# COMPiLELab/krylov_robustness

Measured on AMD Instinct MI355X. Metric: trace(exp(A)) evals/sec + achieved HBM GB/s, n=1M nnz=10M, 1/2/4/8 GPU, higher is better.
Workload: dtype f64

## Files before the change

__graft_entry__.py:

```python
from __future__ import annotations

import os
import subprocess
import sys

ROOT = os.path.dirname(os.path.abspath(__file__))


def build() -> None:
    jobs = str(min(16, os.cpu_count() or 4))
    subprocess.run(["make", "-j", jobs, "-C", os.path.join(ROOT, "krylov_robustness_amd", "csrc")],
                   check=True)
    subprocess.run(["make", "-C", os.path.join(ROOT, "oracle")], check=True)
    subprocess.run(["make", "-j", jobs, "-C", os.path.join(ROOT, "tests", "mexstub")], check=True)
    wave_check = os.path.join(ROOT, "tests", "native", "wave_check")
    if os.path.isfile(os.path.join(wave_check, "Makefile")):
        subprocess.run(["make", "-C", wave_check], check=True)
    if ROOT not in sys.path:
        sys.path.insert(0, ROOT)
    import krylov_robustness_amd as kra
    from krylov_robustness_amd import _lib
    _lib.load()
    assert kra.LIB_PATH.endswith("libkrylov_hip.so")


def smoke() -> None:
    if ROOT not in sys.path:
        sys.path.insert(0, ROOT)
    import numpy as np
    import scipy.sparse as sp

    import krylov_robustness_amd as kra
    from oracle import slq_ref

    z = np.load(os.path.join(ROOT, "tests", "golden", "graphs.npz"))
    n = int(z["oregon_A0__n"][0])
    A = sp.csr_matrix((z["oregon_A0__data"], z["oregon_A0__indices"], z["oregon_A0__indptr"]),
                      shape=(n, n))
    ctx = kra.Context(0)
    D = kra.DeviceMatrix(A, ctx)
    s1, _, q = kra.slq_quadforms(D, 32, 20, seed=7, fun="exp", ctx=ctx)
    _, q_ref = slq_ref.slq_trace(A, 32, 20, seed=7, fun="exp")
    err = float(np.max(np.abs(q - q_ref) / np.abs(q_ref)))
    if not err < 1e-8:
        raise AssertionError(f"smoke: GPU vs oracle max rel err {err:.3e}")
    print(f"smoke ok: tr(exp(A)) ~ {s1 / 32:.6e} (32 probes, m=20), max rel err vs oracle {err:.2e}")


if __name__ == "__main__":
    build()
# ... 3 lines not shown
```

krylov_robustness_amd/csrc/kt_internal.h:

```cpp
#pragma once
#include <algorithm>
#include <hip/hip_runtime.h>
#include <stdint.h>

#include <string>
#include <vector>

#include "../../include/krylov_trace.h"

struct kt_matrix_s;

#ifndef KT_DIAG
#define KT_DIAG 0
#endif

namespace kt {

void set_error(const std::string& msg);

struct Status {
    int code;
    std::string msg;
};

// ... 154 lines not shown
};

}

struct kt_context_s {
    int device = 0;
    hipStream_t stream = nullptr;
    hipStream_t aux_stream[3] = {nullptr, nullptr, nullptr};
    int num_cu = 256;
    bool profile = false;
    int k1_flags = 8;
    bool k2_nt = true;
    int64_t yform_redone = 0;
    int64_t fu_dense = 0;
    int64_t fu_last_cols = 0;
    int64_t expmv_calls = 0;
    int64_t expmv_terms = 0;
    int ky_flags = 8;
    bool yform = true;
    void* blas = nullptr;
    kt_context_s* helper = nullptr;
    void* workers[3] = {nullptr, nullptr, nullptr};
    void (*workers_free)(void*) = nullptr;
    kt::ProfSlot prof[kt::PROF_NSLOTS];
    kt::Workspace ws;
    kt::ScratchPool pool;
};

namespace kt {
struct DevCSR {
    int* rowptr = nullptr;
    int* col = nullptr;
    double* val = nullptr;
    int* long_rows = nullptr;
    int n_long = 0;
    int n_heavy = 0;
    int* med_rows = nullptr;
    int n_med = 0;
    int* short_tasks = nullptr;
    int n_short = 0;
    int* med_tasks = nullptr;
    int* perm = nullptr;
    int *ck_beg = nullptr, *ck_end = nullptr, *sp_rows = nullptr, *sp_first = nullptr;
    int n_chunks = 0, n_split = 0;
    bool built = false;
    char* blob = nullptr;
    size_t blob_bytes = 0;
    PinnedBuf stage;
    void release();
    void invalidate() { built = false; }
};
}

struct kt_matrix_s {
    kt_context_s* ctx = nullptr;
    int64_t n = 0, nnz = 0;
    int long_thresh = 64;
    bool unit_values = false;
    int symmetric = -1;
    kt::DevCSR hub;
    std::vector<int32_t> new2old, old2new;
    kt::DevCSR nat;
    std::vector<int64_t> h_rowptr;
    std::vector<int32_t> h_col;
    std::vector<double> h_val;
    uint64_t version = 0;
// ... 39 lines not shown
```

krylov_robustness_amd/csrc/kt_kernels.hip:

```cpp
#include <hip/hip_runtime.h>

#include "kt_launch.h"
#include "kt_wave.h"
#include <stdint.h>

#include <cstdlib>

#include <type_traits>

namespace kt {

__device__ __forceinline__ uint64_t sm64(uint64_t x) {
    uint64_t z = x + 0x9E3779B97F4A7C15ULL;
    z = (z ^ (z >> 30)) * 0xBF58476D1CE4E5B9ULL;
    z = (z ^ (z >> 27)) * 0x94D049BB133111EBULL;
    return z ^ (z >> 31);
}

template <int P, int VW> struct GeoW {
    static constexpr int VEC = VW;
    static constexpr int LPR = P / VEC;
    static constexpr int GPW = 64 / LPR;
};
template <int P> using Geo = GeoW<P, (P >= 2) ? 2 : 1>;
// ... 354 lines not shown
        guard[p] = 1.0;
    } else {
        const double aj = ys[0 * P + p], bj = ys[1 * P + p], am1 = ys[2 * P + p];
        const double nyj = ys[3 * P + p], ydj = ys[4 * P + p], b1 = ys[5 * P + p];
        g = guard[p];
        const double b1sq = b1 * b1;
        an = (d0 - 2.0 * aj * nyj - 2.0 * bj * ydj + aj * aj * aj + 2.0 * aj * bj * bj + bj * bj * am1) /
             b1sq;
        ny2 = d2;
        bn = b1;
        bnext_sq = ny2 - an * an - b1sq;
        ys[1 * P + p] = b1;
        ys[2 * P + p] = aj;
        ys[4 * P + p] = d1;
    }
    const double bnext = sqrt(fmax(bnext_sq, 0.0));
    ys[0 * P + p] = an;
    ys[3 * P + p] = ny2;
    ys[5 * P + p] = bnext;
    t_alpha[p] = an;
    t_up[p] = bn;
    t_low[p] = bnext;
    if (!last) {
        const double ratio = bnext_sq / ny2;
        guard[p] = (ratio < g || !(ratio == ratio)) ? ratio : g;
    }
    const bool ok = bnext > 0.0 && bnext < INFINITY;
    const double inv = ok ? 1.0 / bnext : 0.0;
    ys[6 * P + p] = inv;
    ys[7 * P + p] = an * inv;
    ys[8 * P + p] = bn * inv;
}

template <int P, int FLAGS, class G = Geo<P>>
__device__ __forceinline__ void row_epilogue_y(int row, int p0, const double* s, const double* cg,
                                               const double* ca, const double* cb, bool has_old,
                                               const double* __restrict__ X,
                                               const double* __restrict__ Yold,
                                               double* __restrict__ Out, double* d0, double* d1,
                                               double* d2, __amdgpu_buffer_rsrc_t orsrc,
                                               const double* __restrict__ Vc = nullptr,
                                               const double* __restrict__ Vo = nullptr,
                                               double* __restrict__ Vn = nullptr, int bcols = 0) {
    using V = VecT<G::VEC>;
    const int64_t off = (int64_t)row * P + p0;
    const typename V::T xi = V::load(X + off);
    if constexpr (FLAGS & KF_VB) {
        if (p0 < bcols) {
            const typename V::T vc = V::load(Vc + off);
            typename V::T vo;
            if (Vo) vo = V::load(Vo + off);
#pragma unroll
            for (int e = 0; e < G::VEC; ++e) {
                double v = fma(-ca[e], V::get(vc, e), cg[e] * V::get(xi, e));
                if (Vo) v = fma(-cb[e], V::get(vo, e), v);
                if (p0 + e < bcols) Vn[off + e] = v;
            }
        }
    }
    if (!Out) {
#pragma unroll
        for (int e = 0; e < G::VEC; ++e) d0[e] = fma(V::get(xi, e), s[e], d0[e]);
        return;
    }
    typename V::T yo;
    if (has_old) yo = V::load_nt(Yold + off);
    typename V::T o;
    double* op = reinterpret_cast<double*>(&o);
#pragma unroll
    for (int e = 0; e < G::VEC; ++e) {
        const double x = V::get(xi, e);
        double u = fma(-ca[e], x, cg[e] * s[e]);
        if (has_old) u = fma(-cb[e], V::get(yo, e), u);
        op[e] = u;
        d0[e] = fma(x, s[e], d0[e]);
        d1[e] = fma(x, u, d1[e]);
        d2[e] = fma(u, u, d2[e]);
    }
    if constexpr (FLAGS & KF_SC1) store_sc1<G::VEC>(orsrc, (uint32_t)(off * 8), op);
    else if constexpr (FLAGS & KF_NTY) V::store_nt(Out + off, o);
    else V::store(Out + off, o);
}

template <int P, class G>
__device__ __forceinline__ double sign_of(uint32_t w, int p0, int e) {
    return ((w >> ((p0 + e) & 31)) & 1u) ? -1.0 : 1.0;
}
template <int P, int FLAGS, class G>
__device__ __forceinline__ void row_gather_signs(int k0, int end, int stride, int p0,
                                                 const int* __restrict__ col,
                                                 const double* __restrict__ val,
                                                 const uint32_t* __restrict__ S, double* s) {
    constexpr int W = (P + 31) / 32;
    const int wo = p0 >> 5;
    int k = k0;
    for (; k + 3 * stride < end; k += 4 * stride) {
        const int c0 = ld_stream<FLAGS>(col + k), c1 = ld_stream<FLAGS>(col + k + stride);
// ... 172 lines not shown
            if (end - beg > long_thresh) continue;
            double s[G::VEC];
#pragma unroll
            for (int e = 0; e < G::VEC; ++e) s[e] = 0.0;
            gather_row<P, FLAGS, G>(beg, end, 1, p0, col, val, X, s);
            row_epilogue_y<P, FLAGS, G>(row, p0, s, cg, ca, cb, has_old, X, Yold, Out, d0, d1, d2,
                                        orsrc, Vc, Vo, Vn, bcols);
        }
    }

#pragma unroll
    for (int o = G::LPR; o < 64; o <<= 1)
#pragma unroll
        for (int e = 0; e < G::VEC; ++e) {
            d0[e] += kt::shfl_xor(d0[e], o);
            d1[e] += kt::shfl_xor(d1[e], o);
            d2[e] += kt::shfl_xor(d2[e], o);
        }
    __shared__ double red[WAVES][3][P];
    if (grp == 0) {
#pragma unroll
        for (int e = 0; e < G::VEC; ++e) {
            red[wave][0][p0 + e] = d0[e];
            red[wave][1][p0 + e] = d1[e];
            red[wave][2][p0 + e] = d2[e];
        }
    }
    __syncthreads();
    for (int t = threadIdx.x; t < 3 * P; t += BLOCK) {
        const int q = t / P, p = t % P;
        double v = 0.0;
#pragma unroll
        for (int w = 0; w < WAVES; ++w) v += red[w][q][p];
        partial[(int64_t)t * gridDim.x + blockIdx.x] = v;
    }
}

template <int P, int BLOCK, int FLAGS>
__global__ __launch_bounds__(BLOCK) void k_spmm_block(
    const int* __restrict__ row_ptr, const int* __restrict__ col, const double* __restrict__ val,
    int n, const double* __restrict__ X, int ldx, double* __restrict__ Y, int ldy,
    const int* __restrict__ long_rows, int n_long, int long_thresh, int long_blocks,
    const int* __restrict__ skip, const int* __restrict__ ck_beg, const int* __restrict__ ck_end,
    int n_chunks, int chunk_blocks, int split_thresh, double* __restrict__ ck_part) {
    using G = GeoB<P>;
    using V = VecT<G::VEC>;
    constexpr int WAVES = BLOCK / 64;
    if (skip && *skip == 0) return;
    X += (int64_t)blockIdx.y * P;
    Y += (int64_t)blockIdx.y * P;
    const int lane = threadIdx.x & 63;
    const int wave = threadIdx.x >> 6;
    const int sub = lane % G::LPR;
    const int grp = lane / G::LPR;
    const int p0 = sub * G::VEC;
    if ((int)blockIdx.x < chunk_blocks) {
        double* part = ck_part + (int64_t)blockIdx.y * n_chunks * P;
        for (int ci = blockIdx.x * WAVES + wave; ci < n_chunks; ci += chunk_blocks * WAVES) {
            double s[G::VEC];
#pragma unroll
            for (int e = 0; e < G::VEC; ++e) s[e] = 0.0;
            gather_row<P, FLAGS, G>(ck_beg[ci] + grp, ck_end[ci], G::GPW, p0, col, val, X, s, ldx);
#pragma unroll
            for (int o = G::LPR; o < 64; o <<= 1)
#pragma unroll
                for (int e = 0; e < G::VEC; ++e) s[e] += kt::shfl_xor(s[e], o);
// ... 1191 lines not shown


hipError_t launch_spmm_lanczos(int P, int flags, int grid, const int* rp, const int* ci,
                               const double* va, int n, const double* X, const double* Yold,
                               double* Out, const double* coef, double* partial,
                               const int* long_rows, int n_long, int long_thresh, int long_blocks,
                               hipStream_t st, const double* Vc, const double* Vo, double* Vn, int bcols) {
    return dispatch_p(P, [&](auto c) {
        constexpr int PP = decltype(c)::value;
#define KT_KY(F)                                                                                   \
    k_spmm_lanczos<PP, kBlock, F><<<grid, kBlock, 0, st>>>(rp, ci, va, n, X, Yold, Out, coef, partial, \
                                                           long_rows, n_long, long_thresh, long_blocks, \
                                                           Vc, Vo, Vn, bcols)
        if (Vn) {
            if (flags & KF_UNIT) {
                if (flags & KF_SC1) KT_KY(KF_UNIT | KF_SC1 | KF_VB);
                else KT_KY(KF_UNIT | KF_VB);
            } else {
                if (flags & KF_SC1) KT_KY(KF_SC1 | KF_VB);
                else KT_KY(KF_VB);
            }
            return;
        }
        switch (flags & (KF_UNIT | KF_NTY | KF_SC1)) {
        case 0: KT_KY(0); break;
        case KF_UNIT: KT_KY(KF_UNIT); break;
        case KF_NTY: KT_KY(KF_NTY); break;
        case KF_UNIT | KF_NTY: KT_KY(KF_UNIT | KF_NTY); break;
        case KF_SC1:
        case KF_SC1 | KF_NTY: KT_KY(KF_SC1); break;
        default: KT_KY(KF_UNIT | KF_SC1); break;
        }
#undef KT_KY
    });
}

hipError_t launch_rademacher_signs(int P, int n, uint64_t seed, int64_t probe_base,
                                  const int* perm, uint32_t* S, hipStream_t st) {
    const int64_t total = (int64_t)n * ((P + 31) / 32);
    int grid = (int)((total + 255) / 256);
    if (grid > 8192) grid = 8192;
    if (grid < 1) grid = 1;
    return dispatch_p(P, [&](auto c) {
        k_rademacher_signs<decltype(c)::value><<<grid, 256, 0, st>>>(n, seed, probe_base, perm, S);
    });
}

hipError_t launch_spmm_lanczos_start(int P, int flags, int grid, const int* rp, const int* ci,
                                     const double* va, int n, const uint32_t* S, double s0,
                                     double* Out, double* partial, const int* long_rows, int n_long,
                                     int long_thresh, int long_blocks, hipStream_t st) {
    return dispatch_p(P, [&](auto c) {
        constexpr int PP = decltype(c)::value;
#define KT_KS(F)                                                                                 \
    k_spmm_lanczos_start<PP, kBlock, F><<<grid, kBlock, 0, st>>>(rp, ci, va, n, S, s0, Out, partial, \
                                                                 long_rows, n_long, long_thresh,  \
                                                                 long_blocks)
        switch (flags & (KF_UNIT | KF_NTY | KF_SC1)) {
        case 0: KT_KS(0); break;
        case KF_UNIT: KT_KS(KF_UNIT); break;
        case KF_NTY: KT_KS(KF_NTY); break;
        case KF_UNIT | KF_NTY: KT_KS(KF_UNIT | KF_NTY); break;
        case KF_SC1:
        case KF_SC1 | KF_NTY: KT_KS(KF_SC1); break;
        default: KT_KS(KF_UNIT | KF_SC1); break;
        }
// ... 260 lines not shown
```

krylov_robustness_amd/csrc/kt_launch.h:

```cpp
#pragma once
#include <hip/hip_runtime.h>
#include <stdint.h>

namespace kt {

int spmm_grid(int n, int P, int max_blocks);
int long_blocks_for(int n_long, int max_blocks);

hipError_t launch_rademacher(int P, int n, uint64_t seed, int64_t probe_base, const int* perm,
                             double* X, hipStream_t st);
hipError_t launch_rademacher_cols(int n, int ncols, uint64_t seed, int64_t probe_base, double* X, int ldx,
                                  hipStream_t st);
hipError_t launch_spmm_dot(int P, int flags, int grid, const int* rp, const int* ci,
                           const double* va, int n, const double* ucur, const double* sc,
                           double* y, double* partial, const int* long_rows, int n_long,
                           int long_thresh, int long_blocks, hipStream_t st);
struct CsrView {
    const int* rp;
    const int* ci;
    const double* va;
    int n;
    const int* long_rows;
    int n_long, long_thresh, split_thresh;
    const int* ck_beg;
// ... 13 lines not shown
constexpr int kMedThresh = 16;
size_t pair_fused_lds_bytes(int it);
bool pairs_dense_eig();
hipError_t launch_pair_fused(int C, int n, int64_t nnz, const CsrView& A, bool unit, const int* ii,
                             const int* jj, const double* B, int it, int fun, double tol, double* vec,
                             double* big, int64_t big_stride, double* state, hipStream_t st);
constexpr int kRegLongCap = 256;
bool pair_reg_applies(int n, int64_t nnz, int it, int n_long, bool unit);
hipError_t launch_pair_reg_dyn(int C, int n, int64_t nnz_max, const CsrView& A, bool unit, const int* ii,
                               const int* jj, const double* B, int it, int fun, double tol, double* state,
                               const int* dyn, hipStream_t st);
hipError_t launch_greedy_edit(int C, const double* state, int* Ti, int* Tj, int nT, int n, int long_thresh,
                              const int* rp, const int* ci, const double* va, const int* lr, const int* dyn,
                              int* rp2, int* ci2, double* va2, int* lr2, int* dyn2, int step, int* sel,
                              double* selv, hipStream_t st);
hipError_t launch_spmm_block(int P, int flags, int grid, const CsrView& M, const double* X, int ldx,
                             double* Y, int ldy, int long_blocks, int chunk_blocks, double* ck_part,
                             hipStream_t st, int slices = 1, const int* skip = nullptr);
hipError_t launch_coef_cgs2(int P, const double* partial, int nblk, int first, const double* k2s,
                            const double* sc, const double* sp, double* coef, double* t_alpha,
                            double* t_up, double* hist, hipStream_t st);
hipError_t launch_update(int P, int grid, int n, const double* y, double* uprev,
                         const double* ucur, const double* sc, const double* sp,
                         const double* coef, int first, double* partial, hipStream_t st,
                         bool nt = false, double* rec = nullptr, int bcols = 0);
hipError_t launch_norm(int P, const double* partial, int nblk, double* k2s, double* scale_next,
                       double* t_low, hipStream_t st);
hipError_t launch_spmm_lanczos(int P, int flags, int grid, const int* rp, const int* ci,
                               const double* va, int n, const double* X, const double* Yold,
                               double* Out, const double* coef, double* partial,
                               const int* long_rows, int n_long, int long_thresh, int long_blocks,
                               hipStream_t st, const double* Vc = nullptr, const double* Vo = nullptr,
                               double* Vn = nullptr, int bcols = 0);
hipError_t launch_rademacher_signs(int P, int n, uint64_t seed, int64_t probe_base,
                                  const int* perm, uint32_t* S, hipStream_t st);
hipError_t launch_spmm_lanczos_start(int P, int flags, int grid, const int* rp, const int* ci,
                                     const double* va, int n, const uint32_t* S, double s0,
                                     double* Out, double* partial, const int* long_rows, int n_long,
                                     int long_thresh, int long_blocks, hipStream_t st);
hipError_t launch_ycoef(int P, const double* partial, int nblk, int start, int last, double s0,
                        double* ys, double* t_alpha, double* t_up, double* t_low, double* guard,
                        hipStream_t st);
hipError_t launch_fill(double* x, int count, double v, hipStream_t st);
hipError_t launch_delay(double microseconds, hipStream_t st);
hipError_t launch_sweep_scales(const double* n2, int nc, int P, int mode, double* a, double* b, hipStream_t st);
hipError_t launch_gram_diag(const double* G, int ld, int nc, double* n2, hipStream_t st);
int gram_ts_chunks(int64_t n);
hipError_t launch_gram_ts(int64_t n, const double* X, int ldx, int px, const double* Y, int ldy, int py,
                          double* part, double* G, hipStream_t st);
hipError_t launch_combine_ts(int64_t n, const double* X, int ldx, int px, const double* C, int q, double alpha,
                             double beta, double* Y, int ldy, hipStream_t st);
hipError_t launch_fro_colmax_scale(int n, double* M, double* out, double* colsq, hipStream_t st);
hipError_t launch_chol_rinv(int bs, const double* G, double shift_coef, double* R, double* Rinv, int* ok,
                            hipStream_t st);
hipError_t launch_scatter_elems(int64_t count, const int64_t* off, const double* val, double* D,
                                hipStream_t st);
hipError_t launch_gather_elems(int64_t count, const double* D, const int64_t* off, double* out,
                               hipStream_t st);
hipError_t launch_gather_rows(int nr, int cols, const double* D, int ldd, const int64_t* rows, double* out,
                              hipStream_t st);
hipError_t launch_weighted_sum(int n, int m, int P, int nc, const double* U, int ldu, int64_t sstride,
                               const double* W, double* Y, int ldy, hipStream_t st);
hipError_t launch_perm_rows(int n, int cols, const int* perm, int gather, const double* src, int lds,
                            double* dst, int ldd, hipStream_t st);
hipError_t launch_axpby(int n, int nc, double a, const double* X, int ldx, double b, double* Y,
                        int ldy, hipStream_t st);
// ... 55 lines not shown
```

krylov_robustness_amd/csrc/kt_runtime.cpp:

```cpp
#include <algorithm>
#include <cstdlib>
#include <cmath>
#include <cstring>
#include <numeric>
#include <string>
#include <thread>

#include <rocblas/rocblas.h>

#include "kt_internal.h"
#include "kt_launch.h"
#include "kt_pool.h"

namespace kt {

static thread_local std::string g_last_error;

void set_error(const std::string& msg) { g_last_error = msg; }

static constexpr unsigned kProfEventFlags = hipEventDisableSystemFence;

void prof_begin(kt_context_s* ctx, int slot, hipStream_t st, int tag) {
    if (!ctx->profile) return;
    ProfSlot& s = ctx->prof[slot];
    if (s.used + 2 > s.ev.size()) {
        for (int i = 0; i < 512; ++i) {
            hipEvent_t e;
            KT_HIP(hipEventCreateWithFlags(&e, kProfEventFlags));
            s.ev.push_back(e);
        }
    }
    if (!s.anchored) {
        if (!s.anchor) KT_HIP(hipEventCreateWithFlags(&s.anchor, kProfEventFlags));
        KT_HIP(hipEventRecord(s.anchor, st ? st : ctx->stream));
        s.anchored = true;
    }
    KT_HIP(hipEventRecord(s.ev[s.used], st ? st : ctx->stream));
    s.tags.push_back(tag);
}

void prof_end(kt_context_s* ctx, int slot, hipStream_t st) {
    if (!ctx->profile) return;
    ProfSlot& s = ctx->prof[slot];
    KT_HIP(hipEventRecord(s.ev[s.used + 1], st ? st : ctx->stream));
// ... 39 lines not shown
            cs = x.first;
            ce = x.second;
            open = true;
        } else if (x.second > ce) {
            ce = x.second;
        }
    }
    if (open) busy += ce - cs;
    return busy;
}

void prof_recycle(kt_context_s* ctx) {
    for (auto& s : ctx->prof) {
        if (s.done == 0) continue;
        std::rotate(s.ev.begin(), s.ev.begin() + (std::ptrdiff_t)s.done, s.ev.begin() + (std::ptrdiff_t)s.used);
        s.used -= s.done;
        s.done = 0;
    }
}

void prof_reserve(kt_context_s* ctx, size_t per_slot) {
    for (auto& s : ctx->prof)
        while (s.ev.size() < per_slot) {
            hipEvent_t e;
            KT_HIP(hipEventCreateWithFlags(&e, kProfEventFlags));
            s.ev.push_back(e);
        }
}

void DevCSR::release() {
    if (blob) (void)hipFree(blob);
    blob = nullptr;
    blob_bytes = 0;
    rowptr = col = long_rows = perm = med_rows = short_tasks = med_tasks = nullptr;
    ck_beg = ck_end = sp_rows = sp_first = nullptr;
    val = nullptr;
    n_long = n_heavy = n_med = n_short = n_chunks = n_split = 0;
    built = false;
}

void build_csr(kt_matrix_s* A, const std::vector<int32_t>& new2old, DevCSR& out, bool sync) {
    const int64_t n = A->n, nnz = A->nnz;
    const bool ident = new2old.empty();
    const bool tasks = ident;
    auto orig = [&](int64_t r) -> int64_t { return ident ? r : new2old[r]; };
    std::vector<int32_t> rp32(n + 1), c32(std::max<int64_t>(nnz, 1));
    std::vector<double> v64(std::max<int64_t>(nnz, 1));
    rp32[0] = 0;
    for (int64_t r = 0; r < n; ++r) {
        const int64_t o = orig(r);
        rp32[r + 1] = rp32[r] + (int32_t)(A->h_rowptr[o + 1] - A->h_rowptr[o]);
    }
    std::vector<std::pair<int32_t, double>> tmp;
    for (int64_t r = 0; r < n; ++r) {
        const int64_t o = orig(r);
        const int64_t kb = A->h_rowptr[o], ke = A->h_rowptr[o + 1];
        if (ident) {
            bool sorted = true;
            for (int64_t k = kb + 1; k < ke && sorted; ++k) sorted = A->h_col[k - 1] < A->h_col[k];
            if (sorted) {
                std::copy(A->h_col.begin() + kb, A->h_col.begin() + ke, c32.begin() + rp32[r]);
                std::copy(A->h_val.begin() + kb, A->h_val.begin() + ke, v64.begin() + rp32[r]);
                continue;
            }
        }
        tmp.clear();
        for (int64_t k = kb; k < ke; ++k)
            tmp.push_back({ident ? A->h_col[k] : A->old2new[A->h_col[k]], A->h_val[k]});
        std::sort(tmp.begin(), tmp.end(), [](const auto& x, const auto& y) { return x.first < y.first; });
        for (size_t t = 0; t < tmp.size(); ++t) {
            c32[rp32[r] + t] = tmp[t].first;
            v64[rp32[r] + t] = tmp[t].second;
        }
    }
    std::vector<int32_t> lr;
    for (int64_t r = 0; r < n; ++r)
        if (rp32[r + 1] - rp32[r] > A->long_thresh) lr.push_back((int32_t)r);
    std::stable_sort(lr.begin(), lr.end(), [&](int32_t a, int32_t b) {
        return rp32[a + 1] - rp32[a] > rp32[b + 1] - rp32[b];
    });
    std::vector<int32_t> mr;
    for (int64_t r = 0; r < n; ++r) {
        const int32_t d = rp32[r + 1] - rp32[r];
        if (d > kMedThresh && d <= A->long_thresh) mr.push_back((int32_t)r);
    }
    std::vector<int32_t> st4;
    if (tasks) {
        const int dmax = std::min(kMedThresh, A->long_thresh);
        const char* sw = std::getenv("KT_EXPMV_SORTWIN");
        const int64_t win = sw ? std::max<int64_t>(0, std::atoll(sw)) : 4096;
        const int64_t W = win > 0 ? win : n;
        std::vector<int64_t> cnt(dmax + 2);
        size_t ns = 0;
        for (int64_t r = 0; r < n; ++r) ns += (rp32[r + 1] - rp32[r] <= dmax);
        st4.assign(4 * ns, 0);
        int64_t t0 = 0;
        for (int64_t w0 = 0; w0 < n; w0 += W) {
            const int64_t w1 = std::min(n, w0 + W);
            std::fill(cnt.begin(), cnt.end(), 0);
            for (int64_t r = w0; r < w1; ++r) {
                const int32_t d = rp32[r + 1] - rp32[r];
                if (d <= dmax) cnt[dmax - d + 1]++;
            }
            cnt[0] = t0;
            for (int i = 1; i <= dmax + 1; ++i) cnt[i] += cnt[i - 1];
// ... 21 lines not shown
    }
    struct Seg {
        void** dst;
        const void* src;
        size_t bytes;
    };
    std::vector<Seg> segs;
    auto add = [&](auto*& dst, const void* src, size_t bytes) {
        segs.push_back({reinterpret_cast<void**>(&dst), src, bytes});
    };
    add(out.rowptr, rp32.data(), sizeof(int) * (n + 1));
    add(out.col, c32.data(), sizeof(int) * c32.size());
    add(out.val, v64.data(), sizeof(double) * v64.size());
    add(out.long_rows, lr.data(), sizeof(int) * lr.size());
    add(out.med_rows, mr.data(), sizeof(int) * mr.size());
    add(out.short_tasks, st4.data(), sizeof(int) * st4.size());
    std::vector<int32_t> mt4;
    if (tasks) {
        mt4.assign(4 * mr.size(), 0);
        for (size_t i = 0; i < mr.size(); ++i) {
            mt4[4 * i] = mr[i];
            mt4[4 * i + 1] = rp32[mr[i]];
            mt4[4 * i + 2] = rp32[mr[i] + 1];
        }
    }
    add(out.med_tasks, mt4.data(), sizeof(int) * mt4.size());
    if (!spr.empty()) {
        add(out.ck_beg, ckb.data(), sizeof(int) * ckb.size());
        add(out.ck_end, cke.data(), sizeof(int) * cke.size());
        add(out.sp_rows, spr.data(), sizeof(int) * spr.size());
        add(out.sp_first, spf.data(), sizeof(int) * spf.size());
    }
    if (!ident) add(out.perm, new2old.data(), sizeof(int) * n);
    auto slice = [](size_t b) { return (std::max<size_t>(b, 16) + 255) & ~(size_t)255; };
    size_t total = 0;
    for (const Seg& g : segs) total += slice(g.bytes);
    KT_HIP(hipStreamSynchronize(A->ctx->stream));
    for (hipStream_t st : A->ctx->aux_stream)
        if (st) KT_HIP(hipStreamSynchronize(st));
    try {
        if (total > out.blob_bytes || !out.blob) {
            if (out.blob) (void)hipFree(out.blob);
            out.blob = nullptr;
            out.blob_bytes = 0;
            KT_HIP(hipMalloc(&out.blob, total));
            out.blob_bytes = total;
        }
        out.stage.ensure(total);
        char* h = out.stage.as<char>();
        size_t off = 0;
        out.ck_beg = out.ck_end = out.sp_rows = out.sp_first = nullptr;
        out.perm = nullptr;
        out.short_tasks = out.med_tasks = nullptr;
        for (const Seg& g : segs) {
            if (g.bytes) std::memcpy(h + off, g.src, g.bytes);
            *g.dst = out.blob + off;
            off += slice(g.bytes);
        }
        KT_HIP(hipMemcpyAsync(out.blob, h, total, hipMemcpyHostToDevice, A->ctx->stream));
        if (sync) KT_HIP(hipStreamSynchronize(A->ctx->stream));
        out.n_long = (int)lr.size();
        out.n_heavy = 0;
        while (out.n_heavy < out.n_long &&
               rp32[lr[out.n_heavy] + 1] - rp32[lr[out.n_heavy]] > kExpmvCoopThresh) ++out.n_heavy;
        out.n_med = (int)mr.size();
        out.n_short = (int)(st4.size() / 4);
        if (!tasks) out.short_tasks = out.med_tasks = nullptr;
        out.n_split = (int)spr.size();
        out.n_chunks = (int)ckb.size();
    } catch (...) {
        out.release();
        throw;
    }
    out.built = true;
}

void refresh_device(kt_matrix_s* A) {
    A->hub.invalidate();
    A->nat.invalidate();
    A->version++;
    A->unit_values = std::all_of(A->h_val.begin(), A->h_val.end(), [](double v) { return v == 1.0; });
}

const DevCSR& hub_csr(kt_matrix_s* A) {
    if (A->hub.built) return A->hub;
    const int64_t n = A->n;
    A->new2old.resize(n);
    A->old2new.resize(n);
    for (int64_t i = 0; i < n; ++i) A->new2old[i] = (int32_t)i;
    std::stable_sort(A->new2old.begin(), A->new2old.end(), [&](int32_t a, int32_t b) {
            return A->h_rowptr[a + 1] - A->h_rowptr[a] > A->h_rowptr[b + 1] - A->h_rowptr[b];
        });
    for (int64_t r = 0; r < n; ++r) A->old2new[A->new2old[r]] = (int32_t)r;
    build_csr(A, A->new2old, A->hub);
    return A->hub;
}

const DevCSR& natural_csr(kt_matrix_s* A) {
    if (!A->nat.built) build_csr(A, std::vector<int32_t>(), A->nat);
    return A->nat;
}

const DevCSR& natural_csr_ordered(kt_matrix_s* A) {
    if (!A->nat.built) build_csr(A, std::vector<int32_t>(), A->nat, false);
    return A->nat;
}

}

using namespace kt;

#define KT_GUARD_BEGIN try {
#define KT_GUARD_END                                   \
    }                                                  \
    catch (const kt::Status& s) {                      \
        kt::set_error(s.msg);                          \
        return s.code;                                 \
    }                                                  \
    catch (const std::bad_alloc&) {                    \
        kt::set_error("host allocation failed");       \
        return KT_ERR_ALLOC;                           \
    }                                                  \
    catch (const std::exception& e) {                  \
        kt::set_error(e.what());                       \
        return KT_ERR_ARG;                             \
// ... 271 lines not shown
```

krylov_robustness_amd/csrc/kt_slq.cpp:

```cpp
#include "kt_slq.h"

#include <algorithm>
#include <chrono>
#include <cstdio>
#include <cmath>
#include <cstdlib>
#include <memory>
#include <thread>

#include "kt_launch.h"
#include "kt_pool.h"

namespace kt {

int slq_auto_block(int64_t n, int64_t nprobes) {
    int P = 128;
    while (P > 8 && (double)n * 8.0 * P > 160.0e6) P >>= 1;
    while (P > 1 && P / 2 >= nprobes) P >>= 1;
    while (P > 16 && nprobes < 2 * P) P >>= 1;
    return P;
}

ExplicitSweep::ExplicitSweep(kt_matrix_s* A_, const DevCSR& M_, int P_, int m_, uint64_t seed_, int64_t probe_base_,
                             const double* x_, int ldx_, int ncols_, const double* dnorms2_, double* rec_host_,
// ... 70 lines not shown
    double* rec = (basis && j + 1 < m) ? bbase + (size_t)(j + 1) * n * bcols : nullptr;
    KT_HIP(launch_update(P, grid, n, Yb, uprev, ucur, sc, sp, coef, first, part2, st, ctx->k2_nt, rec, bcols));
    prof_end(ctx, PROF_UPDATE, st);
    KT_HIP(launch_norm(P, part2, grid, k2s, sn, trec + (size_t)(2 * m + j) * P, st));
    std::swap(ucur, uprev);
    double* t = sp;
    sp = sc;
    sc = sn;
    sn = t;
}

void ExplicitSweep::finish() {
    KT_HIP(hipMemcpyAsync(rec_host, trec, sizeof(double) * (size_t)3 * m * P, hipMemcpyDeviceToHost, st));
    if (scale_hist)
        KT_HIP(hipMemcpyAsync(scale_hist->data(), hist_dev->ptr, sizeof(double) * (size_t)m * P,
                              hipMemcpyDeviceToHost, st));
}

void lanczos_sweep(kt_matrix_s* A, const DevCSR& M, int P, int m, uint64_t seed, int64_t probe_base,
                   const double* x, int ldx, int ncols, const double* dnorms2, double* rec_host,
                   DevMat* basis, std::vector<double>* scale_hist, int lane, int bcols) {
    ExplicitSweep s(A, M, P, m, seed, probe_base, x, ldx, ncols, dnorms2, rec_host, basis, scale_hist, lane, bcols);
    s.start();
    for (int j = 0; j < m; ++j) s.step(j);
    s.finish();
}

YSweep::YSweep(kt_matrix_s* A_, const DevCSR& M_, int P_, int m_, uint64_t seed_, int64_t probe_base_,
               double* rec_host_, int lane_)
    : A(A_), M(M_), P(P_), m(m_), seed(seed_), probe_base(probe_base_), rec_host(rec_host_), lane(lane_) {
    kt_context_s* ctx = A->ctx;
    n = (int)A->n;
    if (lane < 0 || lane > 3) fail(KT_ERR_ARG, "sweep lane out of range");
    if (lane && !ctx->aux_stream[lane - 1])
        KT_HIP(hipStreamCreateWithFlags(&ctx->aux_stream[lane - 1], hipStreamNonBlocking));
    st = lane ? ctx->aux_stream[lane - 1] : ctx->stream;
    grid = spmm_grid(n, P, ctx->num_cu * 4);
    lblocks = long_blocks_for(M.n_long, ctx->num_cu * 2);
    grid1 = grid + lblocks;
    SweepBufs& w = ctx->ws.sweep[lane];
    blk_bytes = sizeof(double) * (size_t)n * P;
    w.X0.ensure(blk_bytes);
    w.X1.ensure(blk_bytes);
    w.Y.ensure(blk_bytes);
    w.partial.ensure(sizeof(double) * (size_t)3 * P * grid1);
    w.coef.ensure(sizeof(double) * 9 * P);
    w.trec.ensure(sizeof(double) * ((size_t)3 * m * P + P));
    part = w.partial.as<double>();
    ys = w.coef.as<double>();
    trec = w.trec.as<double>();
    guard = trec + (size_t)3 * m * P;
    flags = ctx->ky_flags | (A->unit_values ? 2 : 0);
    if (blk_bytes >= ((size_t)1 << 31)) flags &= ~16;
    Z = w.X1.as<uint32_t>();
    Xc = w.Y.as<double>();
    Yo = nullptr;
    Ot = w.X0.as<double>();
}

void YSweep::start() {
    kt_context_s* ctx = A->ctx;
    const double s0 = 1.0 / std::sqrt((double)n);
    KT_HIP(launch_rademacher_signs(P, n, seed, probe_base, M.perm, Z, st));
    prof_begin(ctx, PROF_START, st, P);
    KT_HIP(launch_spmm_lanczos_start(P, flags, grid1, M.rowptr, M.col, M.val, n, Z, s0, Xc, part, M.long_rows,
                                     M.n_long, A->long_thresh, lblocks, st));
    prof_end(ctx, PROF_START, st);
    KT_HIP(launch_ycoef(P, part, grid1, 1, m == 1, s0, ys, rec_at(0, 0), rec_at(1, 0), rec_at(2, 0), guard, st));
}

void YSweep::step(int j) {
    kt_context_s* ctx = A->ctx;
    prof_begin(ctx, PROF_SPMM, st, P);
    const bool last = j + 2 == m;
    KT_HIP(launch_spmm_lanczos(P, flags, grid1, M.rowptr, M.col, M.val, n, Xc, last ? nullptr : Yo,
                               last ? nullptr : Ot, ys + 6 * P, part, M.long_rows, M.n_long, A->long_thresh,
                               lblocks, st));
    prof_end(ctx, PROF_SPMM, st);
    KT_HIP(launch_ycoef(P, part, grid1, 0, last, 0.0, ys, rec_at(0, j + 1), rec_at(1, j + 1), rec_at(2, j + 1),
                        guard, st));
    Yo = Xc;
    Xc = Ot;
    Ot = Yo;
}

void YSweep::finish() {
    KT_HIP(hipMemcpyAsync(rec_host, trec, sizeof(double) * ((size_t)3 * m * P + P), hipMemcpyDeviceToHost, st));
}

YBlockSweep::YBlockSweep(kt_matrix_s* A_, const DevCSR& M_, int P_, int m_, const double* x_, int ldx_, int ncols_,
                         const double* dnorms2_, double* rec_host_, int lane_, double* basis_, int bcols_)
    : A(A_), M(M_), P(P_), m(m_), x(x_), ldx(ldx_), ncols(ncols_), dnorms2(dnorms2_), rec_host(rec_host_),
      lane(lane_), basis(basis_), bcols(basis_ ? bcols_ : 0) {
    kt_context_s* ctx = A->ctx;
    n = (int)A->n;
    if (lane < 0 || lane > 3) fail(KT_ERR_ARG, "sweep lane out of range");
    if (ncols < 1 || ncols > P) fail(KT_ERR_ARG, "y-form block sweep: 1 <= ncols <= P");
    if (lane && !ctx->aux_stream[lane - 1])
        KT_HIP(hipStreamCreateWithFlags(&ctx->aux_stream[lane - 1], hipStreamNonBlocking));
    st = lane ? ctx->aux_stream[lane - 1] : ctx->stream;
    grid = spmm_grid(n, P, ctx->num_cu * 4);
    lblocks = long_blocks_for(M.n_long, ctx->num_cu * 2);
    grid1 = grid + lblocks;
    SweepBufs& w = ctx->ws.sweep[lane];
    blk_bytes = sizeof(double) * (size_t)n * P;
    w.X0.ensure(blk_bytes);
    w.X1.ensure(blk_bytes);
    w.Y.ensure(blk_bytes);
    w.partial.ensure(sizeof(double) * (size_t)3 * P * grid1);
    w.coef.ensure(sizeof(double) * 9 * P);
    w.trec.ensure(sizeof(double) * ((size_t)3 * m * P + P));
    part = w.partial.as<double>();
    ys = w.coef.as<double>();
    trec = w.trec.as<double>();
    guard = trec + (size_t)3 * m * P;
    flags = ctx->ky_flags | (A->unit_values ? 2 : 0);
    if (blk_bytes >= ((size_t)1 << 31)) flags &= ~16;
    V0 = basis ? slot(0) : w.X1.as<double>();
    Xc = w.Y.as<double>();
    Yo = nullptr;
    Ot = w.X0.as<double>();
}

void YBlockSweep::start() {
    KT_HIP(launch_sweep_scales(dnorms2, ncols, P, 1, ys, nullptr, st));
    KT_HIP(hipMemsetAsync(V0, 0, blk_bytes, st));
    KT_HIP(launch_weighted_sum(n, 1, P, ncols, x, ldx, 0, ys, V0, P, st));
    kt_context_s* ctx = A->ctx;
    prof_begin(ctx, PROF_YBLOCK, st, P);
    KT_HIP(launch_spmm_lanczos(P, flags, grid1, M.rowptr, M.col, M.val, n, V0, nullptr, Xc, ys + 6 * P, part,
                               M.long_rows, M.n_long, A->long_thresh, lblocks, st));
    prof_end(ctx, PROF_YBLOCK, st);
    KT_HIP(launch_ycoef(P, part, grid1, 1, m == 1, 1.0, ys, rec_at(0, 0), rec_at(1, 0), rec_at(2, 0), guard, st));
}

void YBlockSweep::step(int j) {
    const bool last = j + 2 == m;
    prof_begin(A->ctx, PROF_YBLOCK, st, P);
    KT_HIP(launch_spmm_lanczos(P, flags, grid1, M.rowptr, M.col, M.val, n, Xc, last ? nullptr : Yo,
                               last ? nullptr : Ot, ys + 6 * P, part, M.long_rows, M.n_long, A->long_thresh, lblocks,
                               st, basis ? slot(j) : nullptr, (basis && j > 0) ? slot(j - 1) : nullptr,
                               basis ? slot(j + 1) : nullptr, bcols));
    prof_end(A->ctx, PROF_YBLOCK, st);
    KT_HIP(launch_ycoef(P, part, grid1, 0, last, 0.0, ys, rec_at(0, j + 1), rec_at(1, j + 1), rec_at(2, j + 1), guard,
                        st));
    Yo = Xc;
    Xc = Ot;
    Ot = Yo;
}

void YBlockSweep::finish() {
    KT_HIP(hipMemcpyAsync(rec_host, trec, sizeof(double) * ((size_t)3 * m * P + P), hipMemcpyDeviceToHost, st));
}

void lanczos_sweep_y_block(kt_matrix_s* A, const DevCSR& M, int P, int m, const double* x, int ldx, int ncols,
                           const double* dnorms2, double* rec_host, int lane) {
    YBlockSweep s(A, M, P, m, x, ldx, ncols, dnorms2, rec_host, lane);
    s.start();
    for (int j = 0; j + 1 < m; ++j) s.step(j);
    s.finish();
}

constexpr double kYformGuard = 1e-4;

int record_tridiag(const double* R, int m, int P, int c, double* al, double* off) {
    int steps = m;
    for (int j = 0; j < m; ++j)
        if (R[(size_t)(2 * m + j) * P + c] < 1e-8) {
            steps = j + 1;
            break;
        }
    for (int j = 0; j < steps; ++j) al[j] = R[(size_t)(0 * m + j) * P + c];
    for (int j = 0; j + 1 < steps; ++j)
        off[j] = 0.5 * (R[(size_t)(2 * m + j) * P + c] + R[(size_t)(1 * m + j + 1) * P + c]);
    return steps;
// ... 418 lines not shown
```

Before: 2.609.

## Use symmetric half-gather quadform kernel for final Lanczos step and hub-aware reordering

For the last Lanczos step, where only the quadratic form x^T A x is needed, a new kernel gathers only the strictly lower-triangular prefix of each row and uses symmetry: it adds 2*s plus the diagonal term. This roughly halves matrix and vector traffic for that step. A per-row 'lower' index array is precomputed on the host and stored with the permuted CSR. Separately, the hub permutation now also groups rows by their first non-hub neighbour rank within degree classes, which is meant to improve locality. The cost is extra host preprocessing and device memory, and a new precondition that the CSR copy carries the lower array.

After: 2.713 (median of 6 runs). +4.0%, better.

```diff
diff --git a/__graft_entry__.py b/__graft_entry__.py
--- a/__graft_entry__.py
+++ b/__graft_entry__.py
@@ -16,6 +16,9 @@
     wave_check = os.path.join(ROOT, "tests", "native", "wave_check")
     if os.path.isfile(os.path.join(wave_check, "Makefile")):
         subprocess.run(["make", "-C", wave_check], check=True)
+    hub_order = os.path.join(ROOT, "tests", "native", "hub_order")
+    if os.path.isfile(os.path.join(hub_order, "Makefile")):
+        subprocess.run(["make", "-C", hub_order], check=True)
     if ROOT not in sys.path:
         sys.path.insert(0, ROOT)
     import krylov_robustness_amd as kra
diff --git a/krylov_robustness_amd/csrc/kt_internal.h b/krylov_robustness_amd/csrc/kt_internal.h
--- a/krylov_robustness_amd/csrc/kt_internal.h
+++ b/krylov_robustness_amd/csrc/kt_internal.h
@@ -210,6 +210,7 @@
     int* rowptr = nullptr;
     int* col = nullptr;
     double* val = nullptr;
+    int* lower = nullptr;
     int* long_rows = nullptr;
     int n_long = 0;
     int n_heavy = 0;
diff --git a/krylov_robustness_amd/csrc/kt_kernels.hip b/krylov_robustness_amd/csrc/kt_kernels.hip
--- a/krylov_robustness_amd/csrc/kt_kernels.hip
+++ b/krylov_robustness_amd/csrc/kt_kernels.hip
@@ -410,6 +410,28 @@
     ys[8 * P + p] = bn * inv;
 }
 
+template <int P, int FLAGS, class G>
+__device__ __forceinline__ void row_basis_y(int64_t off, int p0, const typename VecT<G::VEC>::T& xi,
+                                            const double* cg, const double* ca, const double* cb,
+                                            const double* __restrict__ Vc,
+                                            const double* __restrict__ Vo, double* __restrict__ Vn,
+                                            int bcols) {
+    using V = VecT<G::VEC>;
+    if constexpr (FLAGS & KF_VB) {
+        if (p0 < bcols) {
+            const typename V::T vc = V::load(Vc + off);
+            typename V::T vo;
+            if (Vo) vo = V::load(Vo + off);
+#pragma unroll
+            for (int e = 0; e < G::VEC; ++e) {
+                double v = fma(-ca[e], V::get(vc, e), cg[e] * V::get(xi, e));
+                if (Vo) v = fma(-cb[e], V::get(vo, e), v);
+                if (p0 + e < bcols) Vn[off + e] = v;
+            }
+        }
+    }
+}
+
 template <int P, int FLAGS, class G = Geo<P>>
 __device__ __forceinline__ void row_epilogue_y(int row, int p0, const double* s, const double* cg,
                                                const double* ca, const double* cb, bool has_old,
@@ -423,24 +445,7 @@
     using V = VecT<G::VEC>;
     const int64_t off = (int64_t)row * P + p0;
     const typename V::T xi = V::load(X + off);
-    if constexpr (FLAGS & KF_VB) {
-        if (p0 < bcols) {
-            const typename V::T vc = V::load(Vc + off);
-            typename V::T vo;
-            if (Vo) vo = V::load(Vo + off);
-#pragma unroll
-            for (int e = 0; e < G::VEC; ++e) {
-                double v = fma(-ca[e], V::get(vc, e), cg[e] * V::get(xi, e));
-                if (Vo) v = fma(-cb[e], V::get(vo, e), v);
-                if (p0 + e < bcols) Vn[off + e] = v;
-            }
-        }
-    }
-    if (!Out) {
-#pragma unroll
-        for (int e = 0; e < G::VEC; ++e) d0[e] = fma(V::get(xi, e), s[e], d0[e]);
-        return;
-    }
+    row_basis_y<P, FLAGS, G>(off, p0, xi, cg, ca, cb, Vc, Vo, Vn, bcols);
     typename V::T yo;
     if (has_old) yo = V::load_nt(Yold + off);
     typename V::T o;
@@ -679,6 +684,98 @@
         double v = 0.0;
 #pragma unroll
         for (int w = 0; w < WAVES; ++w) v += red[w][q][p];
+        partial[(int64_t)t * gridDim.x + blockIdx.x] = v;
+    }
+}
+
+template <int P, int BLOCK, int FLAGS>
+__global__ __launch_bounds__(BLOCK) void k_spmm_quadform(
+    const int* __restrict__ row_ptr, const int* __restrict__ col, const double* __restrict__ val,
+    const int* __restrict__ lower, int n, const double* __restrict__ X,
+    const double* __restrict__ coef, double* __restrict__ partial,
+    const int* __restrict__ long_rows, int n_long, int long_thresh, int long_blocks,
+    const double* __restrict__ Vc, const double* __restrict__ Vo, double* __restrict__ Vn, int bcols) {
+    using G = GeoKY<P>;
+    using V = VecT<G::VEC>;
+    constexpr int WAVES = BLOCK / 64;
+    const int lane = threadIdx.x & 63;
+    const int wave = threadIdx.x >> 6;
+    const int sub = lane % G::LPR;
+    const int grp = lane / G::LPR;
+    const int p0 = sub * G::VEC;
+
+    double d0[G::VEC];
+#pragma unroll
+    for (int e = 0; e < G::VEC; ++e) d0[e] = 0.0;
+    double cg[G::VEC], ca[G::VEC], cb[G::VEC];
+    if constexpr (FLAGS & KF_VB) {
+#pragma unroll
+        for (int e = 0; e < G::VEC; ++e) {
+            cg[e] = coef[p0 + e];
+            ca[e] = coef[P + p0 + e];
+            cb[e] = coef[2 * P + p0 + e];
+        }
+    }
+    auto epilogue = [&](int row, int lw, const double* s) {
+        const int64_t off = (int64_t)row * P + p0;
+        const typename V::T xi = V::load(X + off);
+        row_basis_y<P, FLAGS, G>(off, p0, xi, cg, ca, cb, Vc, Vo, Vn, bcols);
+        double arr = 0.0;
+        if (lw < 0) arr = (FLAGS & KF_UNIT) ? 1.0 : val[~lw];
+#pragma unroll
+        for (int e = 0; e < G::VEC; ++e) {
+            const double x = V::get(xi, e);
+            d0[e] = fma(x, fma(2.0, s[e], arr * x), d0[e]);
+        }
+    };
+
+    if ((int)blockIdx.x < long_blocks) {
+        for (int li = blockIdx.x * WAVES + wave; li < n_long; li += long_blocks * WAVES) {
+            const int row = long_rows[li];
+            const int beg = row_ptr[row];
+            const int lw = lower[row];
+            double s[G::VEC];
+#pragma unroll
+            for (int e = 0; e < G::VEC; ++e) s[e] = 0.0;
+            gather_row<P, FLAGS, G>(beg + grp, lw < 0 ? ~lw : lw, G::GPW, p0, col, val, X, s);
+#pragma unroll
+            for (int o = G::LPR; o < 64; o <<= 1)
+#pragma unroll
+                for (int e = 0; e < G::VEC; ++e) s[e] += kt::shfl_xor(s[e], o);
+            if (grp == 0) epilogue(row, lw, s);
+        }
+    } else {
+        const int sb = blockIdx.x - long_blocks;
+        const int groups_total = (gridDim.x - long_blocks) * WAVES * G::GPW;
+        for (int row = (sb * WAVES + wave) * G::GPW + grp; row < n; row += groups_total) {
+            const int beg = row_ptr[row];
+            const int end = row_ptr[row + 1];
+            if (end - beg > long_thresh) continue;
+            const int lw = lower[row];
+            double s[G::VEC];
+#pragma unroll
+            for (int e = 0; e < G::VEC; ++e) s[e] = 0.0;
+            gather_row<P, FLAGS, G>(beg, lw < 0 ? ~lw : lw, 1, p0, col, val, X, s);
+            epilogue(row, lw, s);
+        }
+    }
+
+#pragma unroll
+    for (int o = G::LPR; o < 64; o <<= 1)
+#pragma unroll
+        for (int e = 0; e < G::VEC; ++e) d0[e] += kt::shfl_xor(d0[e], o);
+    __shared__ double red[WAVES][P];
+    if (grp == 0) {
+#pragma unroll
+        for (int e = 0; e < G::VEC; ++e) red[wave][p0 + e] = d0[e];
+    }
+    __syncthreads();
+    for (int t = threadIdx.x; t < 3 * P; t += BLOCK) {
+        double v = 0.0;
+        if (t < P) {
+#pragma unroll
+            for (int w = 0; w < WAVES; ++w) v += red[w][t];
+        }
         partial[(int64_t)t * gridDim.x + blockIdx.x] = v;
     }
 }
@@ -1936,6 +2033,28 @@
         default: KT_KY(KF_UNIT | KF_SC1); break;
         }
 #undef KT_KY
+    });
+}
+
+hipError_t launch_spmm_quadform(int P, int flags, int grid, const int* rp, const int* ci,
+                                const double* va, const int* lower, int n, const double* X,
+                                const double* coef, double* partial, const int* long_rows, int n_long,
+                                int long_thresh, int long_blocks, hipStream_t st, const double* Vc,
+                                const double* Vo, double* Vn, int bcols) {
+    return dispatch_p(P, [&](auto c) {
+        constexpr int PP = decltype(c)::value;
+#define KT_KQ(F)                                                                                    \
+    k_spmm_quadform<PP, kBlock, F><<<grid, kBlock, 0, st>>>(rp, ci, va, lower, n, X, coef, partial, \
+                                                            long_rows, n_long, long_thresh,         \
+                                                            long_blocks, Vc, Vo, Vn, bcols)
+        if (Vn) {
+            if (flags & KF_UNIT) KT_KQ(KF_UNIT | KF_VB);
+            else KT_KQ(KF_VB);
+        } else {
+            if (flags & KF_UNIT) KT_KQ(KF_UNIT);
+            else KT_KQ(0);
+        }
+#undef KT_KQ
     });
 }
 
diff --git a/krylov_robustness_amd/csrc/kt_launch.h b/krylov_robustness_amd/csrc/kt_launch.h
--- a/krylov_robustness_amd/csrc/kt_launch.h
+++ b/krylov_robustness_amd/csrc/kt_launch.h
@@ -69,6 +69,12 @@
                                const int* long_rows, int n_long, int long_thresh, int long_blocks,
                                hipStream_t st, const double* Vc = nullptr, const double* Vo = nullptr,
                                double* Vn = nullptr, int bcols = 0);
+hipError_t launch_spmm_quadform(int P, int flags, int grid, const int* rp, const int* ci,
+                                const double* va, const int* lower, int n, const double* X,
+                                const double* coef, double* partial, const int* long_rows, int n_long,
+                                int long_thresh, int long_blocks, hipStream_t st,
+                                const double* Vc = nullptr, const double* Vo = nullptr,
+                                double* Vn = nullptr, int bcols = 0);
 hipError_t launch_rademacher_signs(int P, int n, uint64_t seed, int64_t probe_base,
                                   const int* perm, uint32_t* S, hipStream_t st);
 hipError_t launch_spmm_lanczos_start(int P, int flags, int grid, const int* rp, const int* ci,
diff --git a/krylov_robustness_amd/csrc/kt_order.h b/krylov_robustness_amd/csrc/kt_order.h
--- /dev/null
+++ b/krylov_robustness_amd/csrc/kt_order.h
@@ -0,0 +1,48 @@
+#pragma once
+#include <algorithm>
+#include <cstdint>
+#include <vector>
+
+namespace kt {
+
+constexpr int64_t kOrderHubRanks = 4096;
+
+inline int64_t order_class(int64_t deg, int long_thresh) { return deg > long_thresh ? deg : (deg + 3) / 4; }
+
+inline void order_counting_sort(const std::vector<int32_t>& idx, const std::vector<int64_t>& key, int64_t nkeys,
+                                std::vector<int32_t>& out) {
+    std::vector<int64_t> cnt((size_t)nkeys + 1, 0);
+    for (int32_t i : idx) cnt[(size_t)key[i] + 1]++;
+    for (int64_t k = 0; k < nkeys; ++k) cnt[(size_t)k + 1] += cnt[(size_t)k];
+    out.resize(idx.size());
+    for (int32_t i : idx) out[(size_t)cnt[(size_t)key[i]]++] = i;
+}
+
+inline void hub_order(int64_t n, const int64_t* rowptr, const int32_t* col, int long_thresh,
+                      std::vector<int32_t>& new2old) {
+    std::vector<int32_t> ident((size_t)n), byrank;
+    std::vector<int64_t> key((size_t)n);
+    int64_t dmax = 0;
+    for (int64_t i = 0; i < n; ++i) {
+        ident[(size_t)i] = (int32_t)i;
+        dmax = std::max(dmax, rowptr[i + 1] - rowptr[i]);
+    }
+    for (int64_t i = 0; i < n; ++i) key[(size_t)i] = dmax - (rowptr[i + 1] - rowptr[i]);
+    order_counting_sort(ident, key, dmax + 1, byrank);
+    std::vector<int32_t> rank((size_t)n);
+    for (int64_t r = 0; r < n; ++r) rank[(size_t)byrank[(size_t)r]] = (int32_t)r;
+    for (int64_t i = 0; i < n; ++i) {
+        int64_t p = n;
+        for (int64_t k = rowptr[i]; k < rowptr[i + 1]; ++k) {
+            const int64_t rc = rank[(size_t)col[k]];
+            if (rc >= kOrderHubRanks && rc < p) p = rc;
+        }
+        key[(size_t)i] = p;
+    }
+    order_counting_sort(ident, key, n + 1, byrank);
+    const int64_t cmax = order_class(dmax, long_thresh);
+    for (int64_t i = 0; i < n; ++i) key[(size_t)i] = cmax - order_class(rowptr[i + 1] - rowptr[i], long_thresh);
+    order_counting_sort(byrank, key, cmax + 1, new2old);
+}
+
+}
diff --git a/krylov_robustness_amd/csrc/kt_runtime.cpp b/krylov_robustness_amd/csrc/kt_runtime.cpp
--- a/krylov_robustness_amd/csrc/kt_runtime.cpp
+++ b/krylov_robustness_amd/csrc/kt_runtime.cpp
@@ -10,6 +10,7 @@
 
 #include "kt_internal.h"
 #include "kt_launch.h"
+#include "kt_order.h"
 #include "kt_pool.h"
 
 namespace kt {
@@ -115,7 +116,7 @@
     if (blob) (void)hipFree(blob);
     blob = nullptr;
     blob_bytes = 0;
-    rowptr = col = long_rows = perm = med_rows = short_tasks = med_tasks = nullptr;
+    rowptr = col = lower = long_rows = perm = med_rows = short_tasks = med_tasks = nullptr;
     ck_beg = ck_end = sp_rows = sp_first = nullptr;
     val = nullptr;
     n_long = n_heavy = n_med = n_short = n_chunks = n_split = 0;
@@ -154,6 +155,17 @@
         for (size_t t = 0; t < tmp.size(); ++t) {
             c32[rp32[r] + t] = tmp[t].first;
             v64[rp32[r] + t] = tmp[t].second;
+        }
+    }
+    std::vector<int32_t> low;
+    if (!ident) {
+        low.resize(n);
+        for (int64_t r = 0; r < n; ++r) {
+            const int32_t* cb = c32.data() + rp32[r];
+            const int32_t* ce = c32.data() + rp32[r + 1];
+            const int32_t* it = std::lower_bound(cb, ce, (int32_t)r);
+            const int32_t k = (int32_t)(it - c32.data());
+            low[r] = (it != ce && *it == (int32_t)r) ? ~k : k;
         }
     }
     std::vector<int32_t> lr;
@@ -241,6 +253,7 @@
         add(out.sp_first, spf.data(), sizeof(int) * spf.size());
     }
     if (!ident) add(out.perm, new2old.data(), sizeof(int) * n);
+    if (!ident) add(out.lower, low.data(), sizeof(int) * n);
     auto slice = [](size_t b) { return (std::max<size_t>(b, 16) + 255) & ~(size_t)255; };
     size_t total = 0;
     for (const Seg& g : segs) total += slice(g.bytes);
@@ -259,7 +272,7 @@
         char* h = out.stage.as<char>();
         size_t off = 0;
         out.ck_beg = out.ck_end = out.sp_rows = out.sp_first = nullptr;
-        out.perm = nullptr;
+        out.perm = out.lower = nullptr;
         out.short_tasks = out.med_tasks = nullptr;
         for (const Seg& g : segs) {
             if (g.bytes) std::memcpy(h + off, g.src, g.bytes);
@@ -294,12 +307,8 @@
 const DevCSR& hub_csr(kt_matrix_s* A) {
     if (A->hub.built) return A->hub;
     const int64_t n = A->n;
-    A->new2old.resize(n);
+    hub_order(n, A->h_rowptr.data(), A->h_col.data(), A->long_thresh, A->new2old);
     A->old2new.resize(n);
-    for (int64_t i = 0; i < n; ++i) A->new2old[i] = (int32_t)i;
-    std::stable_sort(A->new2old.begin(), A->new2old.end(), [&](int32_t a, int32_t b) {
-            return A->h_rowptr[a + 1] - A->h_rowptr[a] > A->h_rowptr[b + 1] - A->h_rowptr[b];
-        });
     for (int64_t r = 0; r < n; ++r) A->old2new[A->new2old[r]] = (int32_t)r;
     build_csr(A, A->new2old, A->hub);
     return A->hub;
diff --git a/krylov_robustness_amd/csrc/kt_slq.cpp b/krylov_robustness_amd/csrc/kt_slq.cpp
--- a/krylov_robustness_amd/csrc/kt_slq.cpp
+++ b/krylov_robustness_amd/csrc/kt_slq.cpp
@@ -126,6 +126,7 @@
     kt_context_s* ctx = A->ctx;
     n = (int)A->n;
     if (lane < 0 || lane > 3) fail(KT_ERR_ARG, "sweep lane out of range");
+    if (!M.lower) fail(KT_ERR_ARG, "y-form sweep: the CSR copy has no lower-prefix array");
     if (lane && !ctx->aux_stream[lane - 1])
         KT_HIP(hipStreamCreateWithFlags(&ctx->aux_stream[lane - 1], hipStreamNonBlocking));
     st = lane ? ctx->aux_stream[lane - 1] : ctx->stream;
@@ -167,9 +168,12 @@
     kt_context_s* ctx = A->ctx;
     prof_begin(ctx, PROF_SPMM, st, P);
     const bool last = j + 2 == m;
-    KT_HIP(launch_spmm_lanczos(P, flags, grid1, M.rowptr, M.col, M.val, n, Xc, last ? nullptr : Yo,
-                               last ? nullptr : Ot, ys + 6 * P, part, M.long_rows, M.n_long, A->long_thresh,
-                               lblocks, st));
+    if (last)
+        KT_HIP(launch_spmm_quadform(P, flags, grid1, M.rowptr, M.col, M.val, M.lower, n, Xc, ys + 6 * P, part,
+                                    M.long_rows, M.n_long, A->long_thresh, lblocks, st));
+    else
+        KT_HIP(launch_spmm_lanczos(P, flags, grid1, M.rowptr, M.col, M.val, n, Xc, Yo, Ot, ys + 6 * P, part,
+                                   M.long_rows, M.n_long, A->long_thresh, lblocks, st));
     prof_end(ctx, PROF_SPMM, st);
     KT_HIP(launch_ycoef(P, part, grid1, 0, last, 0.0, ys, rec_at(0, j + 1), rec_at(1, j + 1), rec_at(2, j + 1),
                         guard, st));
@@ -189,6 +193,7 @@
     kt_context_s* ctx = A->ctx;
     n = (int)A->n;
     if (lane < 0 || lane > 3) fail(KT_ERR_ARG, "sweep lane out of range");
+    if (!M.lower) fail(KT_ERR_ARG, "y-form sweep: the CSR copy has no lower-prefix array");
     if (ncols < 1 || ncols > P) fail(KT_ERR_ARG, "y-form block sweep: 1 <= ncols <= P");
     if (lane && !ctx->aux_stream[lane - 1])
         KT_HIP(hipStreamCreateWithFlags(&ctx->aux_stream[lane - 1], hipStreamNonBlocking));
@@ -231,10 +236,15 @@
 void YBlockSweep::step(int j) {
     const bool last = j + 2 == m;
     prof_begin(A->ctx, PROF_YBLOCK, st, P);
-    KT_HIP(launch_spmm_lanczos(P, flags, grid1, M.rowptr, M.col, M.val, n, Xc, last ? nullptr : Yo,
-                               last ? nullptr : Ot, ys + 6 * P, part, M.long_rows, M.n_long, A->long_thresh, lblocks,
-                               st, basis ? slot(j) : nullptr, (basis && j > 0) ? slot(j - 1) : nullptr,
-                               basis ? slot(j + 1) : nullptr, bcols));
+    const double* vc = basis ? slot(j) : nullptr;
+    const double* vo = (basis && j > 0) ? slot(j - 1) : nullptr;
+    double* vn = basis ? slot(j + 1) : nullptr;
+    if (last)
+        KT_HIP(launch_spmm_quadform(P, flags, grid1, M.rowptr, M.col, M.val, M.lower, n, Xc, ys + 6 * P, part,
+                                    M.long_rows, M.n_long, A->long_thresh, lblocks, st, vc, vo, vn, bcols));
+    else
+        KT_HIP(launch_spmm_lanczos(P, flags, grid1, M.rowptr, M.col, M.val, n, Xc, Yo, Ot, ys + 6 * P, part,
+                                   M.long_rows, M.n_long, A->long_thresh, lblocks, st, vc, vo, vn, bcols));
     prof_end(A->ctx, PROF_YBLOCK, st);
     KT_HIP(launch_ycoef(P, part, grid1, 0, last, 0.0, ys, rec_at(0, j + 1), rec_at(1, j + 1), rec_at(2, j + 1), guard,
                         st));
```
